# ArmingLou/seed-vc

Hardware: AMD Instinct MI355X
Metric: mel_frames_per_sec (higher is better)
Workload: dtype f16; 1 GPU; seed-uvit-tat-xlsr-tiny CFM 25 steps cfg 0.7 + HiFT, batch 64 x (P=430,S=430) per GPU; batch_per_gpu=64, global_batch=64, prompt_frames=430, diffusion_steps=25, vocoder_precision=fp16p8, lanes_per_gpu=2, parallelism=utterance-sharded x1, audio gather on rank 0

## Files before the change

### seed-vc_amd/csrc/common.h

```cpp
#pragma once
#include <atomic>
#include <hip/hip_runtime.h>
#include <stdint.h>
#include <stdio.h>
#include <string>

namespace svc {

typedef _Float16 half_t;
typedef _Float16 half8 __attribute__((ext_vector_type(8)));
typedef _Float16 half4 __attribute__((ext_vector_type(4)));
typedef _Float16 half2v __attribute__((ext_vector_type(2)));
typedef float float4v __attribute__((ext_vector_type(4)));
typedef unsigned int u32x4 __attribute__((ext_vector_type(4)));

void set_error(const std::string& msg);
const char* get_error();

#define SVC_CHECK_HIP(expr)                                                                  \
    do {                                                                                     \
        hipError_t _e = (expr);                                                              \
        if (_e != hipSuccess) {                                                              \
            svc::set_error(std::string(#expr) + ": " + hipGetErrorString(_e) + " at " + __FILE__ + \
                           ":" + std::to_string(__LINE__));                                  \
// ... 35 lines not shown
bool prof_enabled();
void prof_begin(int cls, hipStream_t st);
void prof_end(int cls, double flops, double bytes, hipStream_t st, unsigned long long tag = 0);

template <int MAXA, int DPT>
__device__ __forceinline__ void wait_tiles(int ahead) {
    static_assert(MAXA * DPT <= 63, "vmcnt is a 6-bit counter");
    if constexpr (MAXA <= 0) {
        asm volatile("s_waitcnt vmcnt(0)" ::: "memory");
    } else {
        if (ahead >= MAXA) asm volatile("s_waitcnt vmcnt(%0)" ::"n"(MAXA * DPT) : "memory");
        else wait_tiles<MAXA - 1, DPT>(ahead);
    }
}

__device__ __forceinline__ float act_apply(float v, int act, float slope);
__device__ __forceinline__ uint4 pack8(const float* v) {
    half8 h;
#pragma unroll
    for (int j = 0; j < 8; ++j) h[j] = (half_t)v[j];
    return *reinterpret_cast<uint4*>(&h);
}

static inline int cdiv(long a, long b) { return (int)((a + b - 1) / b); }
static inline long round_up(long a, long b) { return (a + b - 1) / b * b; }

constexpr int KG_MAX_TAPS = 48;

enum { KG_PAD_ZERO = 0, KG_PAD_REFLECT = 1, KG_PAD_CLAMP = 2 };
enum { KG_ACT_NONE = 0, KG_ACT_SILU = 1, KG_ACT_ELU = 2, KG_ACT_LRELU = 3, KG_ACT_TANH = 4, KG_ACT_ABS = 5,
       KG_ACT_CLAMP = 6 , KG_ACT_SIGMOID = 7,
       KG_ACT_GELU = 8  };
enum {
    KG_EPI_STORE = 0,
    KG_EPI_SWIGLU = 1,
    KG_EPI_TANHSIG = 2,
    KG_EPI_QKV_ROPE = 3,
    KG_EPI_STORE_GELU = 4,
};

__device__ __forceinline__ float gelu_erf(float v) { return 0.5f * v * (1.0f + erff(v * 0.70710678118654752f)); }

__device__ __forceinline__ float act_apply(float v, int act, float slope) {
    switch (act) {
        case KG_ACT_SILU: return v / (1.0f + __expf(-v));
        case KG_ACT_ELU: return v > 0.f ? v : (expm1f(v));
        case KG_ACT_LRELU: return v > 0.f ? v : v * slope;
        case KG_ACT_TANH: return tanhf(v);
        case KG_ACT_ABS: return fabsf(v);
        case KG_ACT_CLAMP: return fminf(fmaxf(v, -slope), slope);
        case KG_ACT_SIGMOID: return 1.0f / (1.0f + __expf(-v));
        default: return v;
    }
}

struct KGemmParams {
    const void* a_ptr[KG_MAX_TAPS];
    long a_ld[KG_MAX_TAPS];
    int a_shift[KG_MAX_TAPS];
    int a_ktiles[KG_MAX_TAPS];
    int n_taps;
    int Lout, a_seq_rows, a_off, a_stride, a_len, pad_mode;
    int reflect_min;
    const int* seq_len;
    const void* zero_page;
    float prof_flop_scale;
    int debug;
    int group_n;
    const void* w;
    long ldw;
    int M, N;
    int c_seq_rows, c_off;
    float* c32; long ldc32;
    half_t* c16; long ldc16;
    const float* post_a; const float* post_ib; int post_n; half_t* c16_lo;
    const float* bias;
    const float* rowvec; long ld_rowvec;
    const float* gate;   long ld_gate;
    const float* res;    long ldres;
    const float* res2;   long ldres2;
    float out_scale;
    int act; float act_slope;
    int post_relu;
    int vec_ok;
    const float* rope;
    int rope_D;
    float q_scale;
    half_t* vt; long vt_seq_stride; long vt_ld;
    int vt_mode;
};

int kgemm_launch(const KGemmParams& p, int dtype , int epi, hipStream_t st);
int kgemm_big_launch(const KGemmParams& p, int epi, hipStream_t st);

struct KConvParams {
    const void* a_hi; const void* a_lo;
    const void* w; long ldw;
    const float* bias;
    int B, Lin, Lout, N, cin_pad, k, dil, pad_left, nsub;
    int c_seq_rows, c_off;
    float* c32; long ldc32;
    half_t* c16; half_t* c16_lo; long ldc16;
    const float* post_a; const float* post_ib; int post_n;
    const float* res; long ldres;
    const float* res2; long ldres2;
    float out_scale;
// ... 77 lines not shown
```

### seed-vc_amd/csrc/kconv.hip

```cpp
#include <math.h>
#include <stdlib.h>
#include <string.h>

#include "common.h"

namespace svc {

namespace {

constexpr int CB_NW = 8, CB_NT = CB_NW * 64;
constexpr int CB_SPAN = 64;
constexpr int cb_a_bytes(int bm) { return (bm + CB_SPAN) * 128; }
constexpr int CB_EPI_LD = 68;
constexpr int cb_ns(int bn, int bm) { return bm == 128 ? 2 : (bm < 256 ? 3 : (bn == 128 ? 5 : 8)); }
constexpr int cb_lds(int bn, int bm) { return 2 * cb_a_bytes(bm) + cb_ns(bn, bm) * bn * 128; }

__device__ __forceinline__ int cswz(int row) { return row & 7; }

template <int NSUB, int BN, int BM, bool RAGGED>
__global__ __launch_bounds__(CB_NT, BM < 256 ? 2 : 1) void kconv_kernel(const KConvParams p) {
    constexpr int CB_N = BN, CB_M = BM;
    constexpr int CB_NS = cb_ns(BN, BM);
    constexpr int CB_A_BYTES = cb_a_bytes(BM);
    constexpr int CB_W_BYTES = BN * 128;
// ... 101 lines not shown
                            const int row = wm0 + mt * 16 + fr + shift;
                            const u32x4 x0 = *reinterpret_cast<const u32x4*>(at + row * 128 + ((fq ^ cswz(row)) << 4));
                            const u32x4 x1 = *reinterpret_cast<const u32x4*>(at + row * 128 + (((4 + fq) ^ cswz(row)) << 4));
                            af8[mt] = (v8i){(int)x0[0], (int)x0[1], (int)x0[2], (int)x0[3], (int)x1[0], (int)x1[1], (int)x1[2], (int)x1[3]};
                        }
#pragma unroll
                        for (int nt = 0; nt < 4; ++nt) {
                            const int row = wn0 + nt * 16 + fr;
                            const u32x4 x0 = *reinterpret_cast<const u32x4*>(wt + row * 128 + ((fq ^ cswz(row)) << 4));
                            const u32x4 x1 = *reinterpret_cast<const u32x4*>(wt + row * 128 + (((4 + fq) ^ cswz(row)) << 4));
                            bf8[nt] = (v8i){(int)x0[0], (int)x0[1], (int)x0[2], (int)x0[3], (int)x1[0], (int)x1[1], (int)x1[2], (int)x1[3]};
                        }
                        const int sc_a = 127 - 11, sc_b = 127 - p.w8_exp;
#pragma unroll
                        for (int mt = 0; mt < TM; ++mt)
#pragma unroll
                            for (int nt = 0; nt < 4; ++nt)
                                acc[mt][nt] = __builtin_amdgcn_mfma_scale_f32_16x16x128_f8f6f4(af8[mt], bf8[nt], acc[mt][nt], 0, 0, 0, sc_a, 0, sc_b);
                        stage = stage + 1 == CB_NS ? 0 : stage + 1;
                        fill = fill + 1 == CB_NS ? 0 : fill + 1;
                        continue;
                    }
                }
#pragma unroll
                for (int ks = 0; ks < 2; ++ks) {
                    u32x4 af[TM], bf[4];
                    const int chunk = ks * 4 + fq;
#pragma unroll
                    for (int mt = 0; mt < TM; ++mt) {
                        const int row = wm0 + mt * 16 + fr + shift;
                        af[mt] = *reinterpret_cast<const u32x4*>(at + row * 128 + ((chunk ^ cswz(row)) << 4));
                    }
#pragma unroll
                    for (int nt = 0; nt < 4; ++nt) {
                        const int row = wn0 + nt * 16 + fr;
                        bf[nt] = *reinterpret_cast<const u32x4*>(wt + row * 128 + ((chunk ^ cswz(row)) << 4));
                    }
#pragma unroll
                    for (int mt = 0; mt < TM; ++mt)
#pragma unroll
                        for (int nt = 0; nt < 4; ++nt)
                            acc[mt][nt] = __builtin_amdgcn_mfma_f32_16x16x32_f16(__builtin_bit_cast(half8, af[mt]),
                                                                                 __builtin_bit_cast(half8, bf[nt]), acc[mt][nt], 0, 0, 0);
                }
                stage = stage + 1 == CB_NS ? 0 : stage + 1;
                fill = fill + 1 == CB_NS ? 0 : fill + 1;
            }
        }
    }
    asm volatile("s_waitcnt vmcnt(0)" ::: "memory");
    __syncthreads();

    constexpr int RP = TM >= 2 ? 32 : 16;
    float* ep = reinterpret_cast<float*>(smem) + wave * RP * CB_EPI_LD;
#pragma unroll
    for (int pass = 0; pass < TM * 16 / RP; ++pass) {
        if (pass > 0) __syncthreads();
#pragma unroll
        for (int mi = 0; mi < RP / 16; ++mi)
#pragma unroll
            for (int nt = 0; nt < 4; ++nt)
#pragma unroll
                for (int r = 0; r < 4; ++r)
                    ep[(mi * 16 + fq * 4 + r) * CB_EPI_LD + nt * 16 + fr] = acc[pass * (RP / 16) + mi][nt][r];
        __syncthreads();
#pragma unroll
        for (int i = 0; i < RP / 8; ++i) {
            const int ch = lane + 64 * i;
            const int row = ch >> 3, cc = ch & 7;
            const int pos = p0 + wm0 + pass * RP + row;
            const int n = n0 + wn0 + cc * 8;
            float v[8];
            {
                const float4v x0 = *reinterpret_cast<const float4v*>(ep + row * CB_EPI_LD + cc * 8);
                const float4v x1 = *reinterpret_cast<const float4v*>(ep + row * CB_EPI_LD + cc * 8 + 4);
#pragma unroll
                for (int j = 0; j < 4; ++j) { v[j] = x0[j]; v[4 + j] = x1[j]; }
            }
            if (pos >= p.Lout || n >= p.N) continue;
            const long orow = (long)b * p.c_seq_rows + p.c_off + pos;
            if (p.bias) {
                const float4v b0 = *reinterpret_cast<const float4v*>(p.bias + n);
                const float4v b1 = *reinterpret_cast<const float4v*>(p.bias + n + 4);
#pragma unroll
                for (int j = 0; j < 4; ++j) { v[j] += b0[j]; v[4 + j] += b1[j]; }
            }
            if (p.act != KG_ACT_NONE) {
#pragma unroll
                for (int j = 0; j < 8; ++j) v[j] = act_apply(v[j], p.act, p.act_slope);
            }
            if (p.res) {
                const float4v q0 = *reinterpret_cast<const float4v*>(p.res + orow * p.ldres + n);
                const float4v q1 = *reinterpret_cast<const float4v*>(p.res + orow * p.ldres + n + 4);
#pragma unroll
                for (int j = 0; j < 4; ++j) { v[j] += q0[j]; v[4 + j] += q1[j]; }
            }
            if (p.out_scale != 0.f) {
#pragma unroll
                for (int j = 0; j < 8; ++j) v[j] *= p.out_scale;
            }
            if (p.res2) {
                const float4v q0 = *reinterpret_cast<const float4v*>(p.res2 + orow * p.ldres2 + n);
                const float4v q1 = *reinterpret_cast<const float4v*>(p.res2 + orow * p.ldres2 + n + 4);
#pragma unroll
                for (int j = 0; j < 4; ++j) { v[j] += q0[j]; v[4 + j] += q1[j]; }
            }
            if (p.c32) {
                *reinterpret_cast<float4v*>(p.c32 + orow * p.ldc32 + n) = (float4v){v[0], v[1], v[2], v[3]};
                *reinterpret_cast<float4v*>(p.c32 + orow * p.ldc32 + n + 4) = (float4v){v[4], v[5], v[6], v[7]};
            }
            if (p.post_a) {
                float lo[8];
                float hf[8];
#pragma unroll
                for (int j = 0; j < 8; ++j) {
                    const int nn = n + j;
                    const float sv = nn < p.post_n ? v[j] + p.post_ib[nn] * sin_sq(p.post_a[nn] * v[j]) : 0.f;
                    const half_t hh = (half_t)sv;
                    v[j] = sv;
                    lo[j] = sv - (float)hh;
                    hf[j] = (float)hh;
                }
                if (p.c16_lo) {
                    if (p.c16_lo_fmt) {
                                const u32x4 pr = {lo_pair_p8(hf[0], lo[0]) | (lo_pair_p8(hf[1], lo[1]) << 16), lo_pair_p8(hf[2], lo[2]) | (lo_pair_p8(hf[3], lo[3]) << 16),
                                                  lo_pair_p8(hf[4], lo[4]) | (lo_pair_p8(hf[5], lo[5]) << 16), lo_pair_p8(hf[6], lo[6]) | (lo_pair_p8(hf[7], lo[7]) << 16)};
                                *reinterpret_cast<u32x4*>(p.c16_lo + orow * p.ldc16 + n) = pr;
                            }
                    else *reinterpret_cast<uint4*>(p.c16_lo + orow * p.ldc16 + n) = pack8(lo);
                }
            }
            if (p.c16) *reinterpret_cast<uint4*>(p.c16 + orow * p.ldc16 + n) = pack8(v);
        }
    }
}


__global__ void absmax_kernel(const float* __restrict__ src, int n0, int n1, int n2, long s0, long s1, long s2,
                              const float* __restrict__ scale, float* __restrict__ out) {
    __shared__ float red[256];
    float m = 0.f;
    const long total = (long)n0 * n1 * n2;
    for (long i = (long)blockIdx.x * 256 + threadIdx.x; i < total; i += 256L * gridDim.x) {
        const int i2 = (int)(i % n2);
        const long r = i / n2;
        const int i1 = (int)(r % n1), i0 = (int)(r / n1);
        float v = src[i0 * s0 + i1 * s1 + i2 * s2];
        if (scale) v *= scale[i0];
        m = fmaxf(m, fabsf(v));
    }
    red[threadIdx.x] = m;
    __syncthreads();
    for (int o = 128; o > 0; o >>= 1) {
        if ((int)threadIdx.x < o) red[threadIdx.x] = fmaxf(red[threadIdx.x], red[threadIdx.x + o]);
        __syncthreads();
    }
    if (threadIdx.x == 0) atomicMax(reinterpret_cast<unsigned*>(out), __float_as_uint(red[0]));
}

__global__ void pack_p8_kernel(const float* __restrict__ src, unsigned short* __restrict__ dst, int n0, int n1, int n2, long s0, long s1,
                               long s2, long d0, long d1, long d2, const float* __restrict__ scale, float sw) {
    const long i = (long)blockIdx.x * blockDim.x + threadIdx.x;
    const long total = (long)n0 * n1 * n2;
    if (i >= total) return;
    const int i2 = (int)(i % n2);
    const long r = i / n2;
    const int i1 = (int)(r % n1), i0 = (int)(r / n1);
    float v = src[i0 * s0 + i1 * s1 + i2 * s2];
    if (scale) v *= scale[i0];
    const float hi = (float)(half_t)v, lo = v - hi;
    const float b0 = fminf(fmaxf(lo * sw * 2048.f, -448.f), 448.f), b1 = fminf(fmaxf(hi * sw, -448.f), 448.f);
    dst[i0 * d0 + i1 * d1 + i2 * d2] = (unsigned short)((unsigned)__builtin_amdgcn_cvt_pk_fp8_f32(b0, b1, 0, false) & 0xffffu);
}

}

int kconv_pack_p8(const float* src, unsigned short* dst, int n0, int n1, int n2, long s0, long s1, long s2, long d0, long d1, long d2,
                  const float* scale, int* exp_out, hipStream_t st) {
    float* d_max = nullptr;
    SVC_CHECK_HIP(hipMalloc(&d_max, sizeof(float)));
    SVC_CHECK_HIP(hipMemsetAsync(d_max, 0, sizeof(float), st));
    hipLaunchKernelGGL(absmax_kernel, dim3(256), dim3(256), 0, st, src, n0, n1, n2, s0, s1, s2, scale, d_max);
    float mx = 0.f;
    hipError_t e = hipMemcpyAsync(&mx, d_max, sizeof(float), hipMemcpyDeviceToHost, st);
    if (e == hipSuccess) e = hipStreamSynchronize(st);
// ... 83 lines not shown
```

### seed-vc_amd/csrc/kgemm_tile.h

```cpp
#pragma once
#include <stdlib.h>

#include "common.h"

namespace svc {

namespace {

template <int BM, int BN, int RB, int NS, int NWV>
struct Geo {
    static constexpr int NW = NWV;
    static constexpr int NT = NW * 64;
    static constexpr int WAVES_N = (BN >= 128) ? 2 : 1;
    static constexpr int WAVES_M = NW / WAVES_N;
    static constexpr int WTM = BM / WAVES_M;
    static constexpr int WTN = BN / WAVES_N;
    static constexpr int TM = WTM / 16;
    static constexpr int TN = WTN / 16;
    static constexpr int EPI_LD = WTN + 4;
    static constexpr int NSTAGE = NS;
    static constexpr int STAGE_BYTES = (BM + BN) * RB;
    static constexpr int LDS_AB = NSTAGE * STAGE_BYTES;
    static constexpr int EPI_FULL = NW * WTM * EPI_LD * 4;
    static constexpr int EP = (EPI_FULL <= LDS_AB || TM == 1) ? 1 : ((EPI_FULL / 2 <= LDS_AB || TM == 2) ? 2 : 4);
// ... 296 lines not shown
#undef KG_PIPELOOP
#undef KG_PIPE_STEP
#undef KG_Q
#undef KG_RD_A
#undef KG_RD_B
#undef KG_MAINLOOP
#undef KG_DMA
#undef KG_TAP_SETUP
#undef KG_COMPUTE
#undef KG_CSRC

    if (p.debug & 2) return;
    if constexpr (EPI == KG_EPI_QKV_ROPE) {
        if (v_blk) {
#pragma unroll
            for (int nt = 0; nt < G::TN; ++nt) {
                const int n = n0 + wn0 + CW * (fr >> 2) + 4 * nt + (fr & 3);
                if (n >= p.N) continue;
                const int d = n - 2 * p.rope_D;
#pragma unroll
                for (int mt = 0; mt < G::TM; ++mt) {
                    const int m = m0 + wm0 + mt * 16 + 4 * fq;
                    if (m >= p.M) continue;
                    const int seq = m / p.Lout;
                    const int pos = m - seq * p.Lout;
                    const float4v a4 = KG_ACC(mt, nt);
                    if (m + 4 <= p.M && (pos & 3) == 0 && pos + 4 <= p.Lout) {
                        const half4 h = {(half_t)a4[0], (half_t)a4[1], (half_t)a4[2], (half_t)a4[3]};
                        *reinterpret_cast<half4*>(p.vt + (long)seq * p.vt_seq_stride + (long)d * p.vt_ld + vt_pos(pos, p.vt_mode ? p.vt_mode : 1)) = h;
                    } else {
                        for (int j = 0; j < 4; ++j) {
                            const int mj = m + j;
                            if (mj >= p.M) break;
                            const int sj = mj / p.Lout;
                            const int pj = mj - sj * p.Lout;
                            p.vt[(long)sj * p.vt_seq_stride + (long)d * p.vt_ld + vt_pos(pj, p.vt_mode ? p.vt_mode : 1)] = (half_t)a4[j];
                        }
                    }
                }
            }
            return;
        }
    }

    if constexpr (!DIRECT) {
        __syncthreads();
    constexpr int CW = 8;
    constexpr int CPR = G::WTN / CW;
    constexpr int TMP = G::TM / G::EP;
    constexpr int ROWS_P = TMP * 16;
    constexpr int NCH = ROWS_P * CPR / 64;
    static_assert(ROWS_P * CPR % 64 == 0, "epilogue chunking");
    float* ep = reinterpret_cast<float*>(smem) + wave * ROWS_P * G::EPI_LD;

#pragma unroll
    for (int pass = 0; pass < G::EP; ++pass) {
        const int prow0 = pass * ROWS_P;
        long orow_[NCH];
        int seq_[NCH], pos_[NCH];
        bool ok_[NCH];
        float4v rs0[NCH], rs1[NCH];
#pragma unroll
        for (int i = 0; i < NCH; ++i) {
            const int ch = lane + 64 * i;
            const int row = ch / CPR;
            const int cc = ch - row * CPR;
            const int m = m0 + wm0 + prow0 + row;
            const int n = n0 + wn0 + cc * CW;
            ok_[i] = (m < p.M) & (n < p.N);
            const int mm = ok_[i] ? m : 0;
            seq_[i] = mm / p.Lout;
            pos_[i] = mm - seq_[i] * p.Lout;
            orow_[i] = (long)seq_[i] * p.c_seq_rows + p.c_off + pos_[i];
            rs0[i] = (float4v){0.f, 0.f, 0.f, 0.f};
            rs1[i] = rs0[i];
            {
                if (p.res && p.vec_ok && ok_[i]) {
                    rs0[i] = *reinterpret_cast<const float4v*>(p.res + orow_[i] * p.ldres + n);
                    rs1[i] = *reinterpret_cast<const float4v*>(p.res + orow_[i] * p.ldres + n + 4);
                }
            }
        }
        if (pass > 0) __syncthreads();
#pragma unroll
        for (int mi = 0; mi < TMP; ++mi)
#pragma unroll
            for (int nt = 0; nt < G::TN; ++nt) {
                const float4v a4 = KG_ACC(pass * TMP + mi, nt);
#pragma unroll
                for (int r = 0; r < 4; ++r) ep[(mi * 16 + fq * 4 + r) * G::EPI_LD + nt * 16 + fr] = a4[r];
            }
        __syncthreads();

#pragma unroll
        for (int i = 0; i < NCH; ++i) {
            const int ch = lane + 64 * i;
            const int row = ch / CPR;
            const int cc = ch - row * CPR;
            const int n = n0 + wn0 + cc * CW;
            float v[CW];
#pragma unroll
            for (int q4 = 0; q4 < CW / 4; ++q4) {
                const float4v x = *reinterpret_cast<const float4v*>(ep + row * G::EPI_LD + cc * CW + q4 * 4);
#pragma unroll
                for (int j = 0; j < 4; ++j) v[q4 * 4 + j] = x[j];
            }
            if (!ok_[i]) continue;
            const int seq = seq_[i];
            const int pos = pos_[i];
            const long orow = orow_[i];
            const int nv = (p.N - n) < CW ? (p.N - n) : CW;

            if (p.bias) {
                if (nv == CW) {
#pragma unroll
                    for (int q4 = 0; q4 < CW / 4; ++q4) {
                        const float4v b = *reinterpret_cast<const float4v*>(p.bias + n + q4 * 4);
#pragma unroll
                        for (int j = 0; j < 4; ++j) v[q4 * 4 + j] += b[j];
                    }
                } else {
#pragma unroll
                    for (int j = 0; j < CW; ++j) if (j < nv) v[j] += p.bias[n + j];
                }
            }
            if (p.rowvec) {
                const float* rv = p.rowvec + (long)seq * p.ld_rowvec + n;
#pragma unroll
                for (int j = 0; j < CW; ++j) if (j < nv) v[j] += rv[j];
            }

            {
                if constexpr (EPI == KG_EPI_STORE_GELU) {
#pragma unroll
                    for (int j = 0; j < 8; ++j) v[j] = gelu_erf(v[j]);
                } else if (p.act != KG_ACT_NONE) {
#pragma unroll
                    for (int j = 0; j < 8; ++j) v[j] = act_apply(v[j], p.act, p.act_slope);
                }
                if (p.gate) {
                    const float* gv = p.gate + (long)seq * p.ld_gate + n;
#pragma unroll
                    for (int j = 0; j < 8; ++j) if (j < nv) v[j] *= gv[j];
                }
                if (p.vec_ok) {
                    if (p.res) {
#pragma unroll
                        for (int j = 0; j < 4; ++j) { v[j] += rs0[i][j]; v[4 + j] += rs1[i][j]; }
                    }
                    if (p.out_scale != 0.f) {
#pragma unroll
                        for (int j = 0; j < 8; ++j) v[j] *= p.out_scale;
                    }
                    if (p.res2) {
                        const float4v q0 = *reinterpret_cast<const float4v*>(p.res2 + orow * p.ldres2 + n);
                        const float4v q1 = *reinterpret_cast<const float4v*>(p.res2 + orow * p.ldres2 + n + 4);
#pragma unroll
                        for (int j = 0; j < 4; ++j) { v[j] += q0[j]; v[4 + j] += q1[j]; }
                    }
                    if (p.post_relu) {
#pragma unroll
                        for (int j = 0; j < 8; ++j) v[j] = fmaxf(v[j], 0.f);
                    }
                    if (p.c32) {
                        *reinterpret_cast<float4v*>(p.c32 + orow * p.ldc32 + n) = (float4v){v[0], v[1], v[2], v[3]};
                        *reinterpret_cast<float4v*>(p.c32 + orow * p.ldc32 + n + 4) = (float4v){v[4], v[5], v[6], v[7]};
                    }
                    if (p.post_a) {
                        float lo[8];
#pragma unroll
                        for (int j = 0; j < 8; ++j) {
                            const int nn = n + j;
                            const float sv = nn < p.post_n ? v[j] + p.post_ib[nn] * sin_sq(p.post_a[nn] * v[j]) : 0.f;
                            const half_t h = (half_t)sv;
                            v[j] = sv;
                            lo[j] = sv - (float)h;
                        }
                        if (p.c16_lo) *reinterpret_cast<uint4*>(p.c16_lo + orow * p.ldc16 + n) = pack8(lo);
                    }
                    if (p.c16) *reinterpret_cast<uint4*>(p.c16 + orow * p.ldc16 + n) = pack8(v);
                } else {
                    for (int j = 0; j < nv; ++j) {
                        float o = v[j];
                        if (p.res) o += p.res[orow * p.ldres + n + j];
                        if (p.out_scale != 0.f) o *= p.out_scale;
                        if (p.res2) o += p.res2[orow * p.ldres2 + n + j];
                        if (p.post_relu) o = fmaxf(o, 0.f);
                        if (p.c32) p.c32[orow * p.ldc32 + n + j] = o;
                        if (p.post_a) {
                            const int nn = n + j;
                            o = nn < p.post_n ? o + p.post_ib[nn] * sin_sq(p.post_a[nn] * o) : 0.f;
                            if (p.c16_lo) p.c16_lo[orow * p.ldc16 + n + j] = (half_t)(o - (float)(half_t)o);
                        }
                        if (p.c16) p.c16[orow * p.ldc16 + n + j] = (half_t)o;
                    }
                }
            }
        }
    }
        return;
    }

    const int n = n0 + wn0 + CW * fq;
    if (n >= p.N) return;
    const int nv = (p.N - n) < CW ? (p.N - n) : CW;
    const bool full = nv == CW && p.vec_ok;
    long orow_[G::TM];
    int seq_[G::TM], pos_[G::TM];
    bool ok_[G::TM];
#pragma unroll
    for (int mt = 0; mt < G::TM; ++mt) {
        const int m = m0 + wm0 + mt * 16 + fr;
        ok_[mt] = m < p.M;
        const int mm = ok_[mt] ? m : 0;
        seq_[mt] = mm / p.Lout;
        pos_[mt] = mm - seq_[mt] * p.Lout;
        orow_[mt] = (long)seq_[mt] * p.c_seq_rows + p.c_off + pos_[mt];
    }
    float bias_[CW];
#pragma unroll
    for (int j = 0; j < CW; ++j) bias_[j] = 0.f;
    if (p.bias) {
        if (nv == CW) {
#pragma unroll
            for (int q4 = 0; q4 < CW / 4; ++q4) {
                const float4v b = *reinterpret_cast<const float4v*>(p.bias + n + q4 * 4);
// ... 95 lines not shown
```

### seed-vc_amd/csrc/vocoder.hip

```cpp
#include <math.h>
#include <stdlib.h>
#include <string.h>

#include <algorithm>
#include <vector>

#include "conv_util.h"
#include "noise.h"

using namespace svc;

namespace {


__global__ void snake_params_kernel(const float* alpha, const float* beta, float* a, float* inv_b, int C, int mode) {
    const int c = blockIdx.x * blockDim.x + threadIdx.x;
    if (c >= C) return;
    float al = alpha[c], be = beta ? beta[c] : alpha[c];
    if (mode != 2) { al = expf(al); be = expf(be); }
    a[c] = al;
    inv_b[c] = 1.0f / (be + 1e-9f);
}

template <typename OutT>
// ... 1112 lines not shown
                SVC_CHECK_HIP(hipGetLastError());
            }
            continue;
        }
        if (m->run(mel, f0, phase0, noise, nb, Smb, out, f0_out, st, &rg, seeds)) return 1;
    }
    return 0;
}

extern "C" {

namespace {
thread_local int g_conv1d_took = 0;

int op_conv1d_body(svc_conv1d_ex_t& e, int stride, int pad_mode, bool ex, hipStream_t st) {
    const int B = e.B, L = e.L, Cin = e.Cin, Cout = e.Cout, Lout = e.Lout;
    const int dtype = e.dtype;
    const int c_rows = e.c_rows ? e.c_rows : Lout;
    Arena ar;
    svc_tensor_desc_t d[2];
    d[0].name = "c.weight"; d[0].data = e.w; d[0].ndim = 3; d[0].shape[0] = Cout; d[0].shape[1] = Cin; d[0].shape[2] = e.k; d[0].shape[3] = 1;
    d[1].name = "c.bias"; d[1].data = e.bias; d[1].ndim = 1; d[1].shape[0] = Cout; d[1].shape[1] = d[1].shape[2] = d[1].shape[3] = 1;
    StateDict sd(d, e.bias ? 2 : 1);
    ConvW cw;
    if (pack_conv1d(sd, "c", Cout, Cin, e.k, e.bias != nullptr, dtype, ar, st, &cw)) return 1;
    const size_t n_c = (size_t)B * c_rows * cw.cout_pad;
    float* c = ar.alloc_n<float>(n_c, st);
    if (!c) return 1;
    ConvRun r;
    if (e.a_hi) {
        r.a.hi = e.a_hi; r.a.lo = e.a_lo;
    } else {
        void* a = ar.alloc((size_t)B * L * cw.cin_pad * vesize(dtype), st);
        void* a_lo = ar.alloc((size_t)B * L * cw.cin_pad * vesize(dtype), st);
        if (!a || !a_lo) return 1;
        if (dtype == 3) {
            if (act_cl_launch(e.x, Cin, a, a_lo, cw.cin_pad, 1, nullptr, nullptr, nullptr, B, Cin, L, 2, 1.0f, st, 1)) return 1;
        } else {
            if (pack_any(gdt(dtype), e.x, a, 0, B * L, 1, Cin, Cin, 0, 1, cw.cin_pad, 0, 1, nullptr, st)) return 1;
            if (is_split(dtype))
                if (pack_f16_lo_launch(e.x, (half_t*)a_lo, B * L, 1, Cin, Cin, 0, 1, cw.cin_pad, 0, 1, nullptr, st)) return 1;
        }
        r.a.hi = a; r.a.lo = a_lo;
    }
    r.B = B; r.Lin = L; r.Lout = Lout; r.dilation = e.dilation; r.stride = stride; r.pad_left = e.pad_left; r.pad_mode = pad_mode;
    r.c32 = c; r.ldc32 = cw.cout_pad;
    if (ex) {
        if (pack_f32_launch(e.y, c, B * c_rows, 1, Cout, Cout, 0, 1, cw.cout_pad, 0, 1, nullptr, st)) return 1;
        r.c_rows = e.c_rows; r.c_off = e.c_off;
        r.out_scale = e.out_scale; r.act = e.act; r.act_slope = e.act_slope;
        const float* src[2] = {e.res, e.res2};
        for (int i = 0; i < 2; ++i) {
            if (!src[i]) continue;
            float* q = ar.alloc_n<float>(n_c, st);
            if (!q) return 1;
            if (pack_f32_launch(src[i], q, B * c_rows, 1, Cout, Cout, 0, 1, cw.cout_pad, 0, 1, nullptr, st)) return 1;
            if (i == 0) { r.res = q; r.ldres = cw.cout_pad; } else { r.res2 = q; r.ldres2 = cw.cout_pad; }
        }
        if (e.seq_len) {
            int* d_len = ar.alloc_n<int>(B, st);
            if (!d_len) return 1;
            SVC_CHECK_HIP(hipMemcpyAsync(d_len, e.seq_len, B * sizeof(int), hipMemcpyHostToDevice, st));
            SVC_CHECK_HIP(hipStreamSynchronize(st));
            r.seq_len = d_len; r.seq_kconv = true;
        }
        if (e.post_a) {
            r.post_a = e.post_a; r.post_ib = e.post_ib; r.post_n = Cout;
            r.c16 = reinterpret_cast<half_t*>(e.plane_hi); r.c16_lo = reinterpret_cast<half_t*>(e.plane_lo); r.ldc16 = cw.cout_pad;
            r.c16_lo_fmt = e.next_p8 ? 1 : 0;
        }
        r.p8 = dtype == 3;
        r.bm = e.bm; r.force_gemm = e.force_gemm != 0;
    }
    r.took = &e.took;
    if (conv1d_run(cw, r, st)) return 1;
    g_conv1d_took = e.took;
    if (pack_f32_launch(c, e.y, B * c_rows, 1, Cout, cw.cout_pad, 0, 1, Cout, 0, 1, nullptr, st)) return 1;
    SVC_CHECK_HIP(hipStreamSynchronize(st));
    return 0;
}
}

int svc_op_conv1d(const float* x, const float* w, const float* bias, float* y, int B, int L, int Cin, int Cout, int k,
                  int dilation, int stride, int pad_left, int Lout, int pad_mode, int dtype_in, void* stream) {
    svc_conv1d_ex_t e;
    memset(&e, 0, sizeof(e));
    e.x = x; e.w = w; e.bias = bias; e.y = y;
    e.B = B; e.L = L; e.Cin = Cin; e.Cout = Cout; e.k = k; e.dilation = dilation; e.pad_left = pad_left; e.Lout = Lout;
    e.dtype = dtype_in;
    return op_conv1d_body(e, stride, pad_mode, false, (hipStream_t)stream);
}

int svc_op_conv1d_last_took(void) { return g_conv1d_took; }

int svc_op_conv1d_ex(svc_conv1d_ex_t* e, void* stream) {
    SVC_REQUIRE(e && e->w && e->y && (e->x || e->a_hi), "bad argument");
    SVC_REQUIRE(e->B >= 1 && e->L >= 1 && e->Cin >= 1 && e->Cout >= 1 && e->k >= 1 && e->dilation >= 1 && e->Lout >= 1 && e->pad_left >= 0,
                "svc_op_conv1d_ex: bad shape");
    SVC_REQUIRE(e->dtype == 0 || e->dtype == 2 || e->dtype == 3, "svc_op_conv1d_ex: dtype is 0 (f16), 2 (f16x3) or 3 (fp16 + fp8 corrections)");
    SVC_REQUIRE(e->c_off >= 0 && e->c_off + e->Lout <= (e->c_rows ? e->c_rows : e->Lout), "svc_op_conv1d_ex: the output rows do not fit c_rows");
    SVC_REQUIRE(!e->a_hi || e->dtype == 0 || e->a_lo, "svc_op_conv1d_ex: split operand planes come in pairs");
    SVC_REQUIRE(!e->post_a == !e->post_ib && (!e->post_a || (e->plane_hi && e->plane_lo)), "svc_op_conv1d_ex: the fused Snake needs a, 1/b and both planes");
    SVC_REQUIRE(!e->next_p8 || e->post_a, "svc_op_conv1d_ex: next_p8 selects the format of a fused Snake's lo plane");
    SVC_REQUIRE(!e->force_gemm || (e->dtype != 3 && !e->next_p8), "svc_op_conv1d_ex: the tap-GEMM neither reads nor writes byte-pair planes");
    SVC_REQUIRE(e->bm == 0 || e->bm == 64 || e->bm == 128 || e->bm == 256, "svc_op_conv1d_ex: bm is 0, 64, 128 or 256");
    if (e->seq_len)
        for (int b = 0; b < e->B; ++b) SVC_REQUIRE(e->seq_len[b] >= 0 && e->seq_len[b] <= e->L, "svc_op_conv1d_ex: seq_len out of range");
    e->took = 0;
    return op_conv1d_body(*e, 1, KG_PAD_ZERO, true, (hipStream_t)stream);
// ... 31 lines not shown
```

### seed-vc_amd/ops.py

```python
import torch

from . import _lib


def anti_alias_activation_forward(inputs, up_ftr, down_ftr, alpha, beta):
    assert inputs.is_cuda and inputs.dim() == 3
    x = inputs.contiguous()
    dt = {torch.float32: 0, torch.float16: 1, torch.bfloat16: 2}[x.dtype]
    y = torch.empty_like(x)
    with torch.cuda.device(x.device):
        up = _lib.f32c(up_ftr, x.device).reshape(-1)
        dn = _lib.f32c(down_ftr, x.device).reshape(-1)
        al = _lib.f32c(alpha, x.device).reshape(-1)
        be = _lib.f32c(beta, x.device).reshape(-1)
        B, Cc, L = x.shape
        _lib.check(_lib.lib().svc_anti_alias_act_fwd(_lib.ptr(x), _lib.ptr(y), _lib.ptr(up), _lib.ptr(dn), _lib.ptr(al),
                                                     _lib.ptr(be), B, Cc, L, dt, _lib.stream_ptr()))
    return y


def linear(a, w, bias=None, dtype="f16", act=0):
    M, K = a.shape
    N = w.shape[0]
    dev = a.device
    with torch.cuda.device(dev):
        a, w = _lib.f32c(a), _lib.f32c(w)
        b = _lib.f32c(bias) if bias is not None else None
        c = torch.empty(M, N, device=dev)
        _lib.check(_lib.lib().svc_op_linear(_lib.ptr(a), _lib.ptr(w), _lib.ptr(b), _lib.ptr(c), M, N, K,
                                            0 if dtype == "f16" else 1, act, _lib.stream_ptr()))
    return c


def conv1d_cl(x, w, bias, dilation=1, stride=1, pad_left=0, Lout=None, pad_mode=0, dtype="f32"):
    B, L, Cin = x.shape
    Cout, _, k = w.shape
    dev = x.device
    if Lout is None:
        Lout = L
    with torch.cuda.device(dev):
        x, w = _lib.f32c(x), _lib.f32c(w)
        b = _lib.f32c(bias) if bias is not None else None
        y = torch.empty(B, Lout, Cout, device=dev)
        _lib.check(_lib.lib().svc_op_conv1d(_lib.ptr(x), _lib.ptr(w), _lib.ptr(b), _lib.ptr(y), B, L, Cin, Cout, k,
                                            dilation, stride, pad_left, Lout, pad_mode, {"f16": 0, "f32": 1, "f16x3": 2}[dtype],
                                            _lib.stream_ptr()))
    return y


CONV_DTYPES_EX = {"f16": 0, "f16x3": 2, "p8": 3}
PLANE_FILL = 0x7E7E


def conv1d_cl_ex(x, w, bias=None, dilation=1, pad_left=0, Lout=None, dtype="f16x3", seq_len=None, res=None, res2=None,
                 out_scale=0.0, act=0, act_slope=0.0, c_rows=0, c_off=0, y_fill=None, post_a=None, post_ib=None, next_p8=False,
                 bm=0, force_gemm=False, planes=None):
    import ctypes as C
    B, L, Cin = x.shape
    Cout, _, k = w.shape
    dev = x.device
    if Lout is None:
        Lout = L
    rows = c_rows if c_rows else Lout
    cin_pad, cout_pad = -(-Cin // 64) * 64, -(-Cout // 64) * 64
    with torch.cuda.device(dev):
        e = _lib.Conv1dEx()
        keep = [_lib.f32c(w)]
        e.w = keep[0].data_ptr()
        if planes is not None:
            hi, lo = (p.contiguous() for p in planes)
            assert hi.shape == (B, L, cin_pad) and lo.shape == hi.shape and hi.dtype == torch.int16 and lo.dtype == torch.int16
            keep += [hi, lo]
            e.a_hi, e.a_lo = hi.data_ptr(), lo.data_ptr()
        else:
            keep.append(_lib.f32c(x))
            e.x = keep[-1].data_ptr()
        for name, t, shape in (("bias", bias, (Cout,)), ("res", res, (B, rows, Cout)), ("res2", res2, (B, rows, Cout)),
                               ("post_a", post_a, (Cout,)), ("post_ib", post_ib, (Cout,))):
            if t is not None:
                assert tuple(t.shape) == shape, name
                keep.append(_lib.f32c(t))
                setattr(e, name, keep[-1].data_ptr())
        e.B, e.L, e.Cin, e.Cout, e.k, e.dilation, e.pad_left, e.Lout = B, L, Cin, Cout, k, dilation, pad_left, Lout
        e.dtype = CONV_DTYPES_EX[dtype]
        if seq_len is not None:
            assert len(seq_len) == B
            lens = (C.c_int32 * B)(*[int(v) for v in seq_len])
            e.seq_len = C.cast(lens, C.POINTER(C.c_int32))
        e.out_scale, e.act, e.act_slope, e.c_rows, e.c_off = out_scale, act, act_slope, c_rows, c_off
        e.next_p8, e.bm, e.force_gemm = int(next_p8), bm, int(force_gemm)
        y = torch.full((B, rows, Cout), float("nan") if y_fill is None else y_fill, device=dev)
        e.y = y.data_ptr()
        p_hi = p_lo = None
        if post_a is not None:
            p_hi = torch.full((B, rows, cout_pad), PLANE_FILL, dtype=torch.int16, device=dev)
            p_lo = torch.full((B, rows, cout_pad), PLANE_FILL, dtype=torch.int16, device=dev)
            e.plane_hi, e.plane_lo = p_hi.data_ptr(), p_lo.data_ptr()
        _lib.check(_lib.lib().svc_op_conv1d_ex(C.byref(e), _lib.stream_ptr()))
    return y, p_hi, p_lo, _took(e.took)


def _took(word):
    return {"kconv": bool(word & 1), "bm": (word >> 8) & 0xFFF, "bn": word >> 20}


def conv1d_last_took():
    return _took(_lib.lib().svc_op_conv1d_last_took())


def conv_transpose1d_cl(x, w, bias, stride, dtype="f32"):
    B, L, Cin = x.shape
    _, Cout, k = w.shape
    dev = x.device
    with torch.cuda.device(dev):
        x, w = _lib.f32c(x), _lib.f32c(w)
        b = _lib.f32c(bias) if bias is not None else None
        y = torch.empty(B, L * stride, Cout, device=dev)
        _lib.check(_lib.lib().svc_op_conv_transpose1d(_lib.ptr(x), _lib.ptr(w), _lib.ptr(b), _lib.ptr(y), B, L, Cin, Cout,
                                                      k, stride, {"f16": 0, "f32": 1, "f16x3": 2}[dtype], _lib.stream_ptr()))
    return y


def attention(q, k, v, kv_lens=None):
    N, T, H, hd = q.shape
    assert hd == 64
    dev = q.device
    with torch.cuda.device(dev):
        q, k, v = _lib.f32c(q), _lib.f32c(k), _lib.f32c(v)
        out = torch.empty_like(q)
        lens = _lib.i64_host(kv_lens)
        _lib.check(_lib.lib().svc_op_attention(_lib.ptr(q), _lib.ptr(k), _lib.ptr(v), _lib.ptr(out), N, T, H, lens,
                                               _lib.stream_ptr()))
    return out


def rmsnorm(x, gamma, w=None, b=None, add_one=False):
    rows, D = x.shape
    dev = x.device
    with torch.cuda.device(dev):
        x, gamma = _lib.f32c(x), _lib.f32c(gamma)
        w = _lib.f32c(w) if w is not None else None
        b = _lib.f32c(b) if b is not None else None
        y = torch.empty_like(x)
        _lib.check(_lib.lib().svc_op_rmsnorm(_lib.ptr(x), _lib.ptr(gamma), _lib.ptr(w), _lib.ptr(b), int(add_one),
                                             _lib.ptr(y), rows, D, _lib.stream_ptr()))
# ... 2 lines not shown
```

Before: 135,700 mel-frames/s.

## Hoist epilogue loads, prefetch residuals, and allow in-place residual without repacking

Restructures the conv and GEMM epilogues so each lane owns fixed columns. Bias and snake parameters are loaded once per tile instead of per row, and residual loads are issued before the LDS staging barrier so their latency overlaps it. The activation switch is hoisted out of the 8-element loop, and rowvec and gate reads are vectorised when alignment allows. The vocoder also skips the residual repack copy when the residual aliases the output buffer, and the Python wrapper gains a y_init/'y' path for that case. This adds register pressure from the prefetched residual arrays and relies on the aliased buffer already being in the padded layout.

```diff
diff --git a/seed-vc_amd/csrc/common.h b/seed-vc_amd/csrc/common.h
--- a/seed-vc_amd/csrc/common.h
+++ b/seed-vc_amd/csrc/common.h
@@ -111,6 +111,23 @@
         case KG_ACT_SIGMOID: return 1.0f / (1.0f + __expf(-v));
         default: return v;
     }
+}
+__device__ __forceinline__ void act_apply8(float* v, int act, float slope) {
+#define SVC_ACT8(A)                                                     \
+    case A:                                                             \
+        _Pragma("unroll") for (int j = 0; j < 8; ++j) v[j] = act_apply(v[j], A, slope); \
+        break;
+    switch (act) {
+        SVC_ACT8(KG_ACT_SILU)
+        SVC_ACT8(KG_ACT_ELU)
+        SVC_ACT8(KG_ACT_LRELU)
+        SVC_ACT8(KG_ACT_TANH)
+        SVC_ACT8(KG_ACT_ABS)
+        SVC_ACT8(KG_ACT_CLAMP)
+        SVC_ACT8(KG_ACT_SIGMOID)
+        default: break;
+    }
+#undef SVC_ACT8
 }
 
 struct KGemmParams {
diff --git a/seed-vc_amd/csrc/kconv.hip b/seed-vc_amd/csrc/kconv.hip
--- a/seed-vc_amd/csrc/kconv.hip
+++ b/seed-vc_amd/csrc/kconv.hip
@@ -177,9 +177,42 @@
     __syncthreads();
 
     constexpr int RP = TM >= 2 ? 32 : 16;
+    constexpr int NCH = RP / 8;
     float* ep = reinterpret_cast<float*>(smem) + wave * RP * CB_EPI_LD;
+    const int cc = lane & 7, row0 = lane >> 3;
+    const int n = n0 + wn0 + cc * 8;
+    const bool n_ok = n < p.N;
+    const int n_ld = n_ok ? n : 0;
+    float cb[8], ca[8], cib[8];
+#pragma unroll
+    for (int j = 0; j < 8; ++j) cb[j] = ca[j] = cib[j] = 0.f;
 #pragma unroll
     for (int pass = 0; pass < TM * 16 / RP; ++pass) {
+        bool ok[NCH];
+        long orow[NCH];
+        float4v q[NCH][2], q2[NCH][2];
+#pragma unroll
+        for (int i = 0; i < NCH; ++i) {
+            const int pos = p0 + wm0 + pass * RP + row0 + 8 * i;
+            ok[i] = n_ok & (pos < p.Lout);
+            orow[i] = (long)b * p.c_seq_rows + p.c_off + (ok[i] ? pos : 0);
+        }
+        if (p.res) {
+#pragma unroll
+            for (int i = 0; i < NCH; ++i) {
+                const float* s = p.res + orow[i] * p.ldres + n_ld;
+                q[i][0] = *reinterpret_cast<const float4v*>(s);
+                q[i][1] = *reinterpret_cast<const float4v*>(s + 4);
+            }
+        }
+        if (p.res2) {
+#pragma unroll
+            for (int i = 0; i < NCH; ++i) {
+                const float* s = p.res2 + orow[i] * p.ldres2 + n_ld;
+                q2[i][0] = *reinterpret_cast<const float4v*>(s);
+                q2[i][1] = *reinterpret_cast<const float4v*>(s + 4);
+            }
+        }
         if (pass > 0) __syncthreads();
 #pragma unroll
         for (int mi = 0; mi < RP / 16; ++mi)
@@ -188,13 +221,36 @@
 #pragma unroll
                 for (int r = 0; r < 4; ++r)
                     ep[(mi * 16 + fq * 4 + r) * CB_EPI_LD + nt * 16 + fr] = acc[pass * (RP / 16) + mi][nt][r];
+        if (pass == 0) {
+            if (p.bias) {
+                const float4v b0 = *reinterpret_cast<const float4v*>(p.bias + n_ld);
+                const float4v b1 = *reinterpret_cast<const float4v*>(p.bias + n_ld + 4);
+#pragma unroll
+                for (int j = 0; j < 4; ++j) { cb[j] = b0[j]; cb[4 + j] = b1[j]; }
+            }
+            if (p.post_a && p.post_n > 0) {
+                const bool vec = n_ok && n + 8 <= p.post_n && ((reinterpret_cast<uintptr_t>(p.post_a) | reinterpret_cast<uintptr_t>(p.post_ib)) & 15) == 0;
+                if (vec) {
+                    const float4v a0 = *reinterpret_cast<const float4v*>(p.post_a + n);
+                    const float4v a1 = *reinterpret_cast<const float4v*>(p.post_a + n + 4);
+                    const float4v i0 = *reinterpret_cast<const float4v*>(p.post_ib + n);
+                    const float4v i1 = *reinterpret_cast<const float4v*>(p.post_ib + n + 4);
+#pragma unroll
+                    for (int j = 0; j < 4; ++j) { ca[j] = a0[j]; ca[4 + j] = a1[j]; cib[j] = i0[j]; cib[4 + j] = i1[j]; }
+                } else {
+#pragma unroll
+                    for (int j = 0; j < 8; ++j) {
+                        const int nn = n_ld + j < p.post_n ? n_ld + j : p.post_n - 1;
+                        ca[j] = p.post_a[nn];
+                        cib[j] = p.post_ib[nn];
+                    }
+                }
+            }
+        }
         __syncthreads();
 #pragma unroll
-        for (int i = 0; i < RP / 8; ++i) {
-            const int ch = lane + 64 * i;
-            const int row = ch >> 3, cc = ch & 7;
-            const int pos = p0 + wm0 + pass * RP + row;
-            const int n = n0 + wn0 + cc * 8;
+        for (int i = 0; i < NCH; ++i) {
+            const int row = row0 + 8 * i;
             float v[8];
             {
                 const float4v x0 = *reinterpret_cast<const float4v*>(ep + row * CB_EPI_LD + cc * 8);
@@ -202,45 +258,35 @@
 #pragma unroll
                 for (int j = 0; j < 4; ++j) { v[j] = x0[j]; v[4 + j] = x1[j]; }
             }
-            if (pos >= p.Lout || n >= p.N) continue;
-            const long orow = (long)b * p.c_seq_rows + p.c_off + pos;
+            if (!ok[i]) continue;
             if (p.bias) {
-                const float4v b0 = *reinterpret_cast<const float4v*>(p.bias + n);
-                const float4v b1 = *reinterpret_cast<const float4v*>(p.bias + n + 4);
-#pragma unroll
-                for (int j = 0; j < 4; ++j) { v[j] += b0[j]; v[4 + j] += b1[j]; }
-            }
-            if (p.act != KG_ACT_NONE) {
-#pragma unroll
-                for (int j = 0; j < 8; ++j) v[j] = act_apply(v[j], p.act, p.act_slope);
-            }
+#pragma unroll
+                for (int j = 0; j < 8; ++j) v[j] += cb[j];
+            }
+            if (p.act != KG_ACT_NONE) act_apply8(v, p.act, p.act_slope);
             if (p.res) {
-                const float4v q0 = *reinterpret_cast<const float4v*>(p.res + orow * p.ldres + n);
-                const float4v q1 = *reinterpret_cast<const float4v*>(p.res + orow * p.ldres + n + 4);
-#pragma unroll
-                for (int j = 0; j < 4; ++j) { v[j] += q0[j]; v[4 + j] += q1[j]; }
+#pragma unroll
+                for (int j = 0; j < 4; ++j) { v[j] += q[i][0][j]; v[4 + j] += q[i][1][j]; }
             }
             if (p.out_scale != 0.f) {
 #pragma unroll
                 for (int j = 0; j < 8; ++j) v[j] *= p.out_scale;
             }
             if (p.res2) {
-                const float4v q0 = *reinterpret_cast<const float4v*>(p.res2 + orow * p.ldres2 + n);
-                const float4v q1 = *reinterpret_cast<const float4v*>(p.res2 + orow * p.ldres2 + n + 4);
-#pragma unroll
-                for (int j = 0; j < 4; ++j) { v[j] += q0[j]; v[4 + j] += q1[j]; }
+#pragma unroll
+                for (int j = 0; j < 4; ++j) { v[j] += q2[i][0][j]; v[4 + j] += q2[i][1][j]; }
             }
             if (p.c32) {
-                *reinterpret_cast<float4v*>(p.c32 + orow * p.ldc32 + n) = (float4v){v[0], v[1], v[2], v[3]};
-                *reinterpret_cast<float4v*>(p.c32 + orow * p.ldc32 + n + 4) = (float4v){v[4], v[5], v[6], v[7]};
+                *reinterpret_cast<float4v*>(p.c32 + orow[i] * p.ldc32 + n) = (float4v){v[0], v[1], v[2], v[3]};
+                *reinterpret_cast<float4v*>(p.c32 + orow[i] * p.ldc32 + n + 4) = (float4v){v[4], v[5], v[6], v[7]};
             }
             if (p.post_a) {
                 float lo[8];
                 float hf[8];
 #pragma unroll
                 for (int j = 0; j < 8; ++j) {
-                    const int nn = n + j;
-                    const float sv = nn < p.post_n ? v[j] + p.post_ib[nn] * sin_sq(p.post_a[nn] * v[j]) : 0.f;
+                    const float t = v[j] + cib[j] * sin_sq(ca[j] * v[j]);
+                    const float sv = n + j < p.post_n ? t : 0.f;
                     const half_t hh = (half_t)sv;
                     v[j] = sv;
                     lo[j] = sv - (float)hh;
@@ -250,12 +296,12 @@
                     if (p.c16_lo_fmt) {
                                 const u32x4 pr = {lo_pair_p8(hf[0], lo[0]) | (lo_pair_p8(hf[1], lo[1]) << 16), lo_pair_p8(hf[2], lo[2]) | (lo_pair_p8(hf[3], lo[3]) << 16),
                                                   lo_pair_p8(hf[4], lo[4]) | (lo_pair_p8(hf[5], lo[5]) << 16), lo_pair_p8(hf[6], lo[6]) | (lo_pair_p8(hf[7], lo[7]) << 16)};
-                                *reinterpret_cast<u32x4*>(p.c16_lo + orow * p.ldc16 + n) = pr;
+                                *reinterpret_cast<u32x4*>(p.c16_lo + orow[i] * p.ldc16 + n) = pr;
                             }
-                    else *reinterpret_cast<uint4*>(p.c16_lo + orow * p.ldc16 + n) = pack8(lo);
+                    else *reinterpret_cast<uint4*>(p.c16_lo + orow[i] * p.ldc16 + n) = pack8(lo);
                 }
             }
-            if (p.c16) *reinterpret_cast<uint4*>(p.c16 + orow * p.ldc16 + n) = pack8(v);
+            if (p.c16) *reinterpret_cast<uint4*>(p.c16 + orow[i] * p.ldc16 + n) = pack8(v);
         }
     }
 }
diff --git a/seed-vc_amd/csrc/kgemm_tile.h b/seed-vc_amd/csrc/kgemm_tile.h
--- a/seed-vc_amd/csrc/kgemm_tile.h
+++ b/seed-vc_amd/csrc/kgemm_tile.h
@@ -372,6 +372,17 @@
     constexpr int NCH = ROWS_P * CPR / 64;
     static_assert(ROWS_P * CPR % 64 == 0, "epilogue chunking");
     float* ep = reinterpret_cast<float*>(smem) + wave * ROWS_P * G::EPI_LD;
+    static_assert(64 % CPR == 0, "a lane keeps its columns");
+    const int cc = lane % CPR, row0 = lane / CPR;
+    const int n = n0 + wn0 + cc * CW;
+    const int nv = (p.N - n) < CW ? (p.N - n) : CW;
+    const int n_ld = nv > 0 ? n : 0;
+    const bool rv_vec = p.vec_ok && (p.N & 7) == 0 && (p.ld_rowvec & 3) == 0 && (reinterpret_cast<uintptr_t>(p.rowvec) & 15) == 0;
+    const bool gt_vec = p.vec_ok && (p.N & 7) == 0 && (p.ld_gate & 3) == 0 && (reinterpret_cast<uintptr_t>(p.gate) & 15) == 0;
+    const bool sn_vec = n + CW <= p.post_n && ((reinterpret_cast<uintptr_t>(p.post_a) | reinterpret_cast<uintptr_t>(p.post_ib)) & 15) == 0;
+    float cb[CW];
+#pragma unroll
+    for (int j = 0; j < CW; ++j) cb[j] = 0.f;
 
 #pragma unroll
     for (int pass = 0; pass < G::EP; ++pass) {
@@ -382,23 +393,18 @@
         float4v rs0[NCH], rs1[NCH];
 #pragma unroll
         for (int i = 0; i < NCH; ++i) {
-            const int ch = lane + 64 * i;
-            const int row = ch / CPR;
-            const int cc = ch - row * CPR;
-            const int m = m0 + wm0 + prow0 + row;
-            const int n = n0 + wn0 + cc * CW;
-            ok_[i] = (m < p.M) & (n < p.N);
+            const int m = m0 + wm0 + prow0 + row0 + (64 / CPR) * i;
+            ok_[i] = (m < p.M) & (nv > 0);
             const int mm = ok_[i] ? m : 0;
             seq_[i] = mm / p.Lout;
             pos_[i] = mm - seq_[i] * p.Lout;
             orow_[i] = (long)seq_[i] * p.c_seq_rows + p.c_off + pos_[i];
-            rs0[i] = (float4v){0.f, 0.f, 0.f, 0.f};
-            rs1[i] = rs0[i];
-            {
-                if (p.res && p.vec_ok && ok_[i]) {
-                    rs0[i] = *reinterpret_cast<const float4v*>(p.res + orow_[i] * p.ldres + n);
-                    rs1[i] = *reinterpret_cast<const float4v*>(p.res + orow_[i] * p.ldres + n + 4);
-                }
+        }
+        if (p.res && p.vec_ok) {
+#pragma unroll
+            for (int i = 0; i < NCH; ++i) {
+                rs0[i] = *reinterpret_cast<const float4v*>(p.res + orow_[i] * p.ldres + n_ld);
+                rs1[i] = *reinterpret_cast<const float4v*>(p.res + orow_[i] * p.ldres + n_ld + 4);
             }
         }
         if (pass > 0) __syncthreads();
@@ -410,14 +416,26 @@
 #pragma unroll
                 for (int r = 0; r < 4; ++r) ep[(mi * 16 + fq * 4 + r) * G::EPI_LD + nt * 16 + fr] = a4[r];
             }
+        if (pass == 0 && nv > 0) {
+            if (p.bias) {
+                if (nv == CW) {
+#pragma unroll
+                    for (int q4 = 0; q4 < CW / 4; ++q4) {
+                        const float4v b = *reinterpret_cast<const float4v*>(p.bias + n + q4 * 4);
+#pragma unroll
+                        for (int j = 0; j < 4; ++j) cb[q4 * 4 + j] = b[j];
+                    }
+                } else {
+#pragma unroll
+                    for (int j = 0; j < CW; ++j) if (j < nv) cb[j] = p.bias[n + j];
+                }
+            }
+        }
         __syncthreads();
 
 #pragma unroll
         for (int i = 0; i < NCH; ++i) {
-            const int ch = lane + 64 * i;
-            const int row = ch / CPR;
-            const int cc = ch - row * CPR;
-            const int n = n0 + wn0 + cc * CW;
+            const int row = row0 + (64 / CPR) * i;
             float v[CW];
 #pragma unroll
             for (int q4 = 0; q4 < CW / 4; ++q4) {
@@ -429,25 +447,21 @@
             const int seq = seq_[i];
             const int pos = pos_[i];
             const long orow = orow_[i];
-            const int nv = (p.N - n) < CW ? (p.N - n) : CW;
 
             if (p.bias) {
-                if (nv == CW) {
-#pragma unroll
-                    for (int q4 = 0; q4 < CW / 4; ++q4) {
-                        const float4v b = *reinterpret_cast<const float4v*>(p.bias + n + q4 * 4);
-#pragma unroll
-                        for (int j = 0; j < 4; ++j) v[q4 * 4 + j] += b[j];
-                    }
-                } else {
-#pragma unroll
-                    for (int j = 0; j < CW; ++j) if (j < nv) v[j] += p.bias[n + j];
-                }
+#pragma unroll
+                for (int j = 0; j < CW; ++j) if (j < nv) v[j] += cb[j];
             }
             if (p.rowvec) {
                 const float* rv = p.rowvec + (long)seq * p.ld_rowvec + n;
-#pragma unroll
-                for (int j = 0; j < CW; ++j) if (j < nv) v[j] += rv[j];
+                if (rv_vec) {
+                    const float4v rv0 = *reinterpret_cast<const float4v*>(rv), rv1 = *reinterpret_cast<const float4v*>(rv + 4);
+#pragma unroll
+                    for (int j = 0; j < 4; ++j) { v[j] += rv0[j]; v[4 + j] += rv1[j]; }
+                } else {
+#pragma unroll
+                    for (int j = 0; j < CW; ++j) if (j < nv) v[j] += rv[j];
+                }
             }
 
             {
@@ -455,13 +469,18 @@
 #pragma unroll
                     for (int j = 0; j < 8; ++j) v[j] = gelu_erf(v[j]);
                 } else if (p.act != KG_ACT_NONE) {
-#pragma unroll
-                    for (int j = 0; j < 8; ++j) v[j] = act_apply(v[j], p.act, p.act_slope);
+                    act_apply8(v, p.act, p.act_slope);
                 }
                 if (p.gate) {
                     const float* gv = p.gate + (long)seq * p.ld_gate + n;
-#pragma unroll
-                    for (int j = 0; j < 8; ++j) if (j < nv) v[j] *= gv[j];
+                    if (gt_vec) {
+                        const float4v gt0 = *reinterpret_cast<const float4v*>(gv), gt1 = *reinterpret_cast<const float4v*>(gv + 4);
+#pragma unroll
+                        for (int j = 0; j < 4; ++j) { v[j] *= gt0[j]; v[4 + j] *= gt1[j]; }
+                    } else {
+#pragma unroll
+                        for (int j = 0; j < 8; ++j) if (j < nv) v[j] *= gv[j];
+                    }
                 }
                 if (p.vec_ok) {
                     if (p.res) {
@@ -487,11 +506,27 @@
                         *reinterpret_cast<float4v*>(p.c32 + orow * p.ldc32 + n + 4) = (float4v){v[4], v[5], v[6], v[7]};
                     }
                     if (p.post_a) {
-                        float lo[8];
+                        float lo[8], ca[8], cib[8];
+                        if (sn_vec) {
+#pragma unroll
+                            for (int q4 = 0; q4 < 2; ++q4) {
+                                const float4v a4 = *reinterpret_cast<const float4v*>(p.post_a + n + q4 * 4);
+                                const float4v i4 = *reinterpret_cast<const float4v*>(p.post_ib + n + q4 * 4);
+#pragma unroll
+                                for (int j = 0; j < 4; ++j) { ca[q4 * 4 + j] = a4[j]; cib[q4 * 4 + j] = i4[j]; }
+                            }
+                        } else {
+#pragma unroll
+                            for (int j = 0; j < 8; ++j) {
+                                const int nn = n + j < p.post_n ? n + j : (p.post_n > 0 ? p.post_n - 1 : 0);
+                                ca[j] = p.post_n > 0 ? p.post_a[nn] : 0.f;
+                                cib[j] = p.post_n > 0 ? p.post_ib[nn] : 0.f;
+                            }
+                        }
 #pragma unroll
                         for (int j = 0; j < 8; ++j) {
-                            const int nn = n + j;
-                            const float sv = nn < p.post_n ? v[j] + p.post_ib[nn] * sin_sq(p.post_a[nn] * v[j]) : 0.f;
+                            const float t = v[j] + cib[j] * sin_sq(ca[j] * v[j]);
+                            const float sv = n + j < p.post_n ? t : 0.f;
                             const half_t h = (half_t)sv;
                             v[j] = sv;
                             lo[j] = sv - (float)h;
diff --git a/seed-vc_amd/csrc/vocoder.hip b/seed-vc_amd/csrc/vocoder.hip
--- a/seed-vc_amd/csrc/vocoder.hip
+++ b/seed-vc_amd/csrc/vocoder.hip
@@ -1188,9 +1188,12 @@
         const float* src[2] = {e.res, e.res2};
         for (int i = 0; i < 2; ++i) {
             if (!src[i]) continue;
-            float* q = ar.alloc_n<float>(n_c, st);
-            if (!q) return 1;
-            if (pack_f32_launch(src[i], q, B * c_rows, 1, Cout, Cout, 0, 1, cw.cout_pad, 0, 1, nullptr, st)) return 1;
+            float* q = c;
+            if (src[i] != e.y) {
+                q = ar.alloc_n<float>(n_c, st);
+                if (!q) return 1;
+                if (pack_f32_launch(src[i], q, B * c_rows, 1, Cout, Cout, 0, 1, cw.cout_pad, 0, 1, nullptr, st)) return 1;
+            }
             if (i == 0) { r.res = q; r.ldres = cw.cout_pad; } else { r.res2 = q; r.ldres2 = cw.cout_pad; }
         }
         if (e.seq_len) {
diff --git a/seed-vc_amd/ops.py b/seed-vc_amd/ops.py
--- a/seed-vc_amd/ops.py
+++ b/seed-vc_amd/ops.py
@@ -54,7 +54,7 @@
 
 def conv1d_cl_ex(x, w, bias=None, dilation=1, pad_left=0, Lout=None, dtype="f16x3", seq_len=None, res=None, res2=None,
                  out_scale=0.0, act=0, act_slope=0.0, c_rows=0, c_off=0, y_fill=None, post_a=None, post_ib=None, next_p8=False,
-                 bm=0, force_gemm=False, planes=None):
+                 bm=0, force_gemm=False, planes=None, y_init=None):
     import ctypes as C
     B, L, Cin = x.shape
     Cout, _, k = w.shape
@@ -77,7 +77,7 @@
             e.x = keep[-1].data_ptr()
         for name, t, shape in (("bias", bias, (Cout,)), ("res", res, (B, rows, Cout)), ("res2", res2, (B, rows, Cout)),
                                ("post_a", post_a, (Cout,)), ("post_ib", post_ib, (Cout,))):
-            if t is not None:
+            if t is not None and not isinstance(t, str):
                 assert tuple(t.shape) == shape, name
                 keep.append(_lib.f32c(t))
                 setattr(e, name, keep[-1].data_ptr())
@@ -89,8 +89,16 @@
             e.seq_len = C.cast(lens, C.POINTER(C.c_int32))
         e.out_scale, e.act, e.act_slope, e.c_rows, e.c_off = out_scale, act, act_slope, c_rows, c_off
         e.next_p8, e.bm, e.force_gemm = int(next_p8), bm, int(force_gemm)
-        y = torch.full((B, rows, Cout), float("nan") if y_fill is None else y_fill, device=dev)
+        if y_init is not None:
+            assert tuple(y_init.shape) == (B, rows, Cout)
+            y = _lib.f32c(y_init).clone()
+        else:
+            y = torch.full((B, rows, Cout), float("nan") if y_fill is None else y_fill, device=dev)
         e.y = y.data_ptr()
+        for name, t in (("res", res), ("res2", res2)):
+            if isinstance(t, str):
+                assert t == "y" and y_init is not None, name
+                setattr(e, name, e.y)
         p_hi = p_lo = None
         if post_a is not None:
             p_hi = torch.full((B, rows, cout_pad), PLANE_FILL, dtype=torch.int16, device=dev)
```

Result: faster. 138,300 mel-frames/s, median of 6 (+1.9%).
